# sara-nl/saraGAN

Hardware: AMD Instinct MI355X
Metric: 3D volumes/sec/node (G+D step) at 128x128x32 (higher is better)
Workload: dtype bf16

## Files before the change

### saragan_amd/csrc/common.h

```cpp
#pragma once
#include <hip/hip_runtime.h>
#include <stdint.h>
#include <mutex>
#include "../../include/saragan_hip.h"

typedef __bf16 bf16_t;
typedef float f32x4 __attribute__((ext_vector_type(4)));
typedef float f32x16 __attribute__((ext_vector_type(16)));
typedef __bf16 bf16x8 __attribute__((ext_vector_type(8)));
typedef __bf16 bf16x4 __attribute__((ext_vector_type(4)));
typedef short s16x4 __attribute__((ext_vector_type(4)));
typedef uint32_t u32x4 __attribute__((ext_vector_type(4)));

#define SG_STORE16_GUARD(v) asm volatile("s_nop 1" ::"v"(v))
typedef uint32_t u32x2 __attribute__((ext_vector_type(2)));

#define SG_LAUNCH_CHECK()                          \
  do {                                             \
    hipError_t e__ = hipGetLastError();            \
    if (e__ != hipSuccess) return (int)e__;        \
  } while (0)

static inline hipStream_t sg_st(sg_stream_t s) { return (hipStream_t)s; }

struct sg_config {
  int fwd_lds, fwd_tg;
  int fwd_v1, fwd_no_pw, fwd_no_dense;
  int fwd_no_v3, fwd_no_v3s, fwd_no_v4, fwd_no_v5, fwd_no_ksplit;
  int fwd3p_16;
  int fwd3s_16;
  int fwd_no_3p;
  int fwd3_gx, fwd3_no_lean;
  int fwd4_gx, fwd4_no_lean, fwd4_no_wres;
  int wgrad_v1, wgrad_no_v3, wgrad_no_lean;
  int wgrad_no_w16;
  int wgrad3l_min_cols;
  int wgrad3l_16;
  int wgrad_v1_blocks;
  int dbg_flags;
  int no_small;
  int deterministic;
  int gemm_ks_model;
  int gemm_k333_maxvox;
  int no_gemm;
};
const sg_config& sg_cfg();

bool sg_gemm_conv_eligible(const sg_conv_shape* s, sg_dtype dt);
size_t sg_gemm_conv_workspace(const sg_conv_shape* s, sg_dtype dt);
int sg_gemm_conv_fwd(const void* x, const void* wp, void* y, const sg_conv_shape* s, const float* bias, int act, float slope,
                     const uint32_t* mask_bits, float mask_slope, uint32_t* sign_out, void* workspace, size_t workspace_bytes,
                     hipStream_t st, bool* used);

bool sg_small_eligible(const sg_conv_shape* s);
bool sg_small_wgrad_eligible(const sg_conv_shape* s);
size_t sg_small_tail_bytes(const sg_conv_shape* s);
size_t sg_small_wgrad_workspace(const sg_conv_shape* s);
int sg_small_pack(const float* w, float coef, int flip, void* tail, const sg_conv_shape* s, sg_dtype dt, hipStream_t st);
int sg_small_fwd(const void* x, const void* tail, void* y, const sg_conv_shape* s, const float* bias, int act, float slope,
                 int pixel_norm, float eps, float* pn_scale, const uint32_t* mask_bits, float mask_slope, uint32_t* sign_out,
                 sg_dtype dt, hipStream_t st);
int sg_small_wgrad(const void* x, const void* dy, float* dw, float* dbias, float coef, void* workspace, size_t workspace_bytes,
                   const sg_conv_shape* s, sg_dtype dt, hipStream_t st);

#define SG_ALLOW_160K_LDS(kern)                                                                                  \
  do {                                                                                                           \
    static std::once_flag once__;                                                                                \
    static hipError_t err__ = hipSuccess;                                                                        \
    std::call_once(once__, [&] {                                                                                 \
      err__ = hipFuncSetAttribute((const void*)(kern), hipFuncAttributeMaxDynamicSharedMemorySize, 160 * 1024);  \
    });                                                                                                          \
    if (err__ != hipSuccess) return (int)err__;                                                                  \
  } while (0)
static inline size_t sg_esize(sg_dtype dt) { return dt == SG_BF16 ? 2 : 4; }
static inline bool sg_aligned16(const void* p) { return (((uintptr_t)p) & 15) == 0; }

__device__ __forceinline__ void philox4x32_10(uint32_t c0, uint32_t c1, uint32_t c2, uint32_t c3, uint32_t k0,
                                              uint32_t k1, uint32_t out[4]) {
#pragma unroll
  for (int rnd = 0; rnd < 10; ++rnd) {
    const uint32_t hi0 = __umulhi(0xD2511F53u, c0), lo0 = 0xD2511F53u * c0;
    const uint32_t hi1 = __umulhi(0xCD9E8D57u, c2), lo1 = 0xCD9E8D57u * c2;
    const uint32_t n0 = hi1 ^ c1 ^ k0, n1 = lo1, n2 = hi0 ^ c3 ^ k1, n3 = lo0;
    c0 = n0; c1 = n1; c2 = n2; c3 = n3;
    k0 += 0x9E3779B9u; k1 += 0xBB67AE85u;
  }
  out[0] = c0; out[1] = c1; out[2] = c2; out[3] = c3;
}

struct sg_fastdiv {
  uint32_t d, m;
};
static inline __host__ __device__ sg_fastdiv sg_make_fastdiv(uint32_t d) {
  sg_fastdiv f;
  f.d = d;
  f.m = d <= 1 ? 0u : (uint32_t)((0x100000000ull + d - 1) / d);
  return f;
}
__device__ __forceinline__ uint32_t sg_div(uint32_t x, sg_fastdiv f) {
  return f.d <= 1 ? x : __umulhi(x, f.m);
}

template <typename T>
struct sg_traits;
template <>
struct sg_traits<float> {
  static constexpr int CH = 8;
  __device__ static __forceinline__ float to_f(float v) { return v; }
  __device__ static __forceinline__ float from_f(float v) { return v; }
};
template <>
struct sg_traits<bf16_t> {
  static constexpr int CH = 16;
  __device__ static __forceinline__ float to_f(bf16_t v) { return (float)v; }
  __device__ static __forceinline__ bf16_t from_f(float v) { return (bf16_t)v; }
};

template <typename T>
__device__ __forceinline__ f32x16 sg_mfma_chunk(u32x4 a, u32x4 b, f32x16 c);
template <>
// ... 201 lines not shown
```

### saragan_amd/csrc/prof.hip

```cpp
#include "prof.h"
#include <mutex>
#include <vector>
#include <string.h>
#include <stdlib.h>
#include <atomic>

namespace {
struct Rec { int kind; sg_conv_shape shape; int dtype; hipEvent_t e0, e1; bool ok; const char* name; };
std::mutex g_mu;
bool g_on = false;
bool g_filter = false;
int g_fkind = 0;
sg_conv_shape g_fshape;
std::vector<Rec> g_recs;
const char* kVersion = "saragan_hip 0.4 (gfx950)";
}

bool sg_prof_on() { return g_on; }
thread_local const char* sg_tls_kernel = "";

namespace {
std::atomic<const sg_config*> g_cfg{nullptr};
int env_int(const char* name, int dflt) {
  const char* v = getenv(name);
  return v && *v ? atoi(v) : dflt;
}
const sg_config* read_config() {
  sg_config* c = new sg_config;
  c->fwd_lds = env_int("SG_FWD_LDS", 80 * 1024);
  c->fwd_tg = env_int("SG_FWD_TG", 0);
  c->fwd_v1 = env_int("SG_FWD_V1", 0);
  c->fwd_no_pw = env_int("SG_FWD_NO_PW", 0);
  c->fwd_no_dense = env_int("SG_FWD_NO_DENSE", 0);
  c->fwd_no_v3 = env_int("SG_FWD_NO_V3", 0);
  c->fwd_no_v3s = env_int("SG_FWD_NO_V3S", 0);
  c->wgrad_no_lean = env_int("SG_WGRAD_NO_LEAN", 0);
  c->wgrad_no_w16 = env_int("SG_WGRAD_NO_W16", 0);
  c->wgrad3l_16 = env_int("SG_WGRAD3L_16", 0);
  c->wgrad3l_min_cols = env_int("SG_WGRAD3L_MIN_COLS", 0);
  c->wgrad_v1_blocks = env_int("SG_WGRAD_V1_BLOCKS", 0);
  c->fwd_no_v4 = env_int("SG_FWD_NO_V4", 0);
  c->fwd_no_v5 = env_int("SG_FWD_NO_V5", 0);
  c->fwd_no_ksplit = env_int("SG_FWD_NO_KSPLIT", 0);
  c->fwd_no_3p = env_int("SG_FWD_NO_3P", 0);
  c->fwd3p_16 = env_int("SG_FWD3P_16", 1);
  c->fwd3s_16 = env_int("SG_FWD3S_16", 1);
  c->fwd3_gx = env_int("SG_FWD3_GX", 0);
  c->fwd3_no_lean = env_int("SG_FWD3_NO_LEAN", 0);
  c->fwd4_gx = env_int("SG_FWD4_GX", 0);
  c->fwd4_no_lean = env_int("SG_FWD4_NO_LEAN", 0);
  c->fwd4_no_wres = env_int("SG_FWD4_NO_WRES", 0);
  c->wgrad_v1 = env_int("SG_WGRAD_V1", 0);
  c->wgrad_no_v3 = env_int("SG_WGRAD_NO_V3", 0);
  c->dbg_flags = env_int("SG_DBG_FLAGS", 0);
  c->no_small = env_int("SG_NO_SMALL", 0);
  c->deterministic = env_int("SG_DETERMINISTIC", 0);
  c->no_gemm = env_int("SG_NO_GEMM", 0);
  c->gemm_ks_model = env_int("SG_GEMM_KS_MODEL", 0);
  c->gemm_k333_maxvox = env_int("SG_GEMM_K333_MAXVOX", 8192);
  return c;
}
}

const sg_config& sg_cfg() {
  const sg_config* c = g_cfg.load(std::memory_order_acquire);
  if (c == nullptr) {
    std::lock_guard<std::mutex> lk(g_mu);
    c = g_cfg.load(std::memory_order_acquire);
    if (c == nullptr) {
      c = read_config();
      g_cfg.store(c, std::memory_order_release);
    }
  }
  return *c;
}

extern "C" int sg_config_reload(void) {
  std::lock_guard<std::mutex> lk(g_mu);
  g_cfg.store(read_config(), std::memory_order_release);
  return SG_OK;
}

void sg_prof_begin(int kind, const sg_conv_shape* s, sg_dtype dt, hipStream_t st, int* slot) {
  std::lock_guard<std::mutex> lk(g_mu);
  if (g_filter && (kind != g_fkind || memcmp(s, &g_fshape, sizeof(sg_conv_shape)) != 0)) { *slot = -1; return; }
  Rec r; r.kind = kind; r.shape = *s; r.dtype = (int)dt; r.ok = false; r.name = "";
  if (hipEventCreate(&r.e0) != hipSuccess) { *slot = -1; return; }
  if (hipEventCreate(&r.e1) != hipSuccess) { (void)hipEventDestroy(r.e0); *slot = -1; return; }
  (void)hipEventRecord(r.e0, st);
  g_recs.push_back(r);
  *slot = (int)g_recs.size() - 1;
}

void sg_prof_end(int slot, hipStream_t st) {
  std::lock_guard<std::mutex> lk(g_mu);
  bool ok = slot >= 0;
  int idx = ok ? slot : -1 - slot;
  if (idx < 0 || idx >= (int)g_recs.size()) return;
  (void)hipEventRecord(g_recs[idx].e1, st);
  g_recs[idx].ok = ok;
}

void sg_prof_name(int slot, const char* name) {
  std::lock_guard<std::mutex> lk(g_mu);
  if (slot >= 0 && slot < (int)g_recs.size()) g_recs[slot].name = name;
}

extern "C" const char* sg_version(void) { return kVersion; }

extern "C" const char* sg_error_string(int code) {
  switch (code) {
    case SG_OK: return "ok";
    case SG_EINVAL: return "invalid argument (shape, null pointer or unsupported combination)";
    case SG_EWORKSPACE: return "workspace too small";
    case SG_EALIGN: return "pointer not 16-byte aligned";
    case SG_EUNSUPPORTED: return "no kernel covers this request";
    default: break;
  }
  if (code > 0) return hipGetErrorString((hipError_t)code);
  return "unknown error";
}
// ... 53 lines not shown
```

### saragan_amd/csrc/wgrad.hip

```cpp
#include "common.h"
#include "prof.h"
#include <stdlib.h>
#include <type_traits>

struct WgradArgs {
  const void* x;
  const void* dy;
  float* dwt;
  sg_tile_geom g;
  sg_tile_geom gy;
  int cin, cout, taps, kh, kw, tap0, taps_blk;
  int ciT, coT;
  int rs;
  int xbytes, ybytes;
  int ntiles;
  sg_fastdiv fnp;
  int vec_x, vec_y;
  int plane_rows;
  float* dbias;
  int64_t slab, bslab;
  int nslab;
  int dbg_flags;
  unsigned long long* dbg;
  const uint32_t* dy_mask;
// ... 967 lines not shown
  template <int I>
  static __device__ __forceinline__ void prologue(const Ctx& c, frag_t (&a0)[RING], frag_t (&a1)[RING], frag_t (&b0)[2],
                                                  frag_t (&b1)[2]) {
    if constexpr (I < PF && I < NI) {
      load<I>(c, a0, a1, b0, b1);
      prologue<I + 1>(c, a0, a1, b0, b1);
    }
  }
  static __device__ __forceinline__ void run(const Ctx& c, f32x16 (&acc)[MAXT]) {
    frag_t a0[RING], a1[RING], b0[2], b1[2];
    SG_KLOOP_BEGIN();
    prologue<0>(c, a0, a1, b0, b1);
    step<0>(c, acc, a0, a1, b0, b1);
    SG_KLOOP_END();
  }
};

template <int PF, int TW = 32>
struct sg_wgrad_tile_lean16 {
  static constexpr int MAXT = 7, TH = 128 / TW, HW = TW + 2, RPS = 32 / TW;
  static constexpr int NKS = 8, IPS = 2 + 2 * MAXT, NI = NKS * IPS, RING = PF + 1;
  static_assert(PF * 2 + 2 <= 15, "lgkmcnt is a 4-bit counter");
  typedef s16x4 frag_t;
  struct Ctx {
    int xb[2][MAXT];
    int yb;
  };
  struct HF { frag_t p[2]; };
  template <int I>
  static __device__ __forceinline__ void load(const Ctx& c, HF (&a)[RING], HF (&b)[2][2]) {
    constexpr int ks = I / IPS, r = I % IPS, td = ks / (NKS / 2), th = (ks % (NKS / 2)) * RPS;
    if constexpr (r < 2) {
      asm volatile("ds_read_b64_tr_b16 %0, %1 offset:%2" : "=v"(b[ks & 1][r].p[0]) : "v"(c.yb), "n"(ks * 2048 + r * 32));
      asm volatile("ds_read_b64_tr_b16 %0, %1 offset:%2" : "=v"(b[ks & 1][r].p[1]) : "v"(c.yb), "n"(ks * 2048 + r * 32 + 256));
    } else {
      constexpr int t = r - 2, j = t / 2, h = t % 2, SL = (ks * 2 * MAXT + t) % RING;
      constexpr int off = th * HW * 64 + h * 32;
      asm volatile("ds_read_b64_tr_b16 %0, %1 offset:%2" : "=v"(a[SL].p[0]) : "v"(c.xb[td][j]), "n"(off));
      asm volatile("ds_read_b64_tr_b16 %0, %1 offset:%2" : "=v"(a[SL].p[1]) : "v"(c.xb[td][j]), "n"(off + 256));
    }
  }
  static __device__ __forceinline__ u32x4 cat(const HF& f) {
    u32x4 o;
    o[0] = __builtin_bit_cast(u32x2, f.p[0])[0]; o[1] = __builtin_bit_cast(u32x2, f.p[0])[1];
    o[2] = __builtin_bit_cast(u32x2, f.p[1])[0]; o[3] = __builtin_bit_cast(u32x2, f.p[1])[1];
    return o;
  }
  template <int I>
  static __device__ __forceinline__ void step(const Ctx& c, f32x4 (&acc)[MAXT][4], HF (&a)[RING], HF (&b)[2][2]) {
    if constexpr (I < NI) {
      if constexpr (I + PF < NI) load<I + PF>(c, a, b);
      constexpr int ks = I / IPS, r = I % IPS;
      if constexpr (r >= 2) {
        constexpr int younger = (NI - 1 - I < PF ? NI - 1 - I : PF) * 2;
        asm volatile("s_waitcnt lgkmcnt(%0)" ::"n"(younger));
        __builtin_amdgcn_sched_barrier(0);
        constexpr int t = r - 2, j = t / 2, h = t % 2, SL = (ks * 2 * MAXT + t) % RING;
        const u32x4 af = cat(a[SL]);
#pragma unroll
        for (int hb = 0; hb < 2; ++hb)
          acc[j][h * 2 + hb] = __builtin_amdgcn_mfma_f32_16x16x32_bf16(__builtin_bit_cast(bf16x8, af), __builtin_bit_cast(bf16x8, cat(b[ks & 1][hb])),
                                                                       acc[j][h * 2 + hb], 0, 0, 0);
        __builtin_amdgcn_sched_barrier(0);
      }
      step<I + 1>(c, acc, a, b);
    }
  }
  template <int I>
  static __device__ __forceinline__ void prologue(const Ctx& c, HF (&a)[RING], HF (&b)[2][2]) {
    if constexpr (I < PF && I < NI) {
      load<I>(c, a, b);
      prologue<I + 1>(c, a, b);
    }
  }
  static __device__ __forceinline__ void run(const Ctx& c, f32x4 (&acc)[MAXT][4]) {
    HF a[RING], b[2][2];
    SG_KLOOP_BEGIN();
    prologue<0>(c, a, b);
    step<0>(c, acc, a, b);
    SG_KLOOP_END();
  }
};

template <bool UPS, bool DYM = false, int TW = 32, bool M16 = false>
__global__ __launch_bounds__(512) void conv_wgrad3l_kernel(WgradArgs a) {
  static_assert(!(UPS && DYM), "one gathered operand at a time");
  static_assert(TW == 32 || TW == 16, "tile width");
  extern __shared__ __attribute__((aligned(16))) char smem[];
  constexpr int TAPS = 27, MAXT = 7;
  constexpr int TH = 128 / TW, HH = TH + 2, HW = TW + 2, PB = 208 * 64, XB = 4 * PB, YB = 256 * 64, BUF = XB + YB;
  static_assert(HH * HW <= 208, "halo plane slot");
  constexpr int XPIECES = (HH * HW + 15) / 16;
  constexpr int ONES_OFF = 2 * BUF, ONES_BYTES = 12288;
  static_assert((TH - 1) * HW * 64 + 2304 + 1024 + 12 * 64 + 64 <= ONES_BYTES, "ones image covers every fragment offset");
  for (int i = threadIdx.x * 16; i < ONES_BYTES; i += 512 * 16)
    *reinterpret_cast<u32x4*>(smem + ONES_OFF + i) = u32x4{0x3F803F80u, 0x3F803F80u, 0x3F803F80u, 0x3F803F80u};
  constexpr uint32_t DEAD = 0x80000000u;
  const sg_tile_geom& g = a.g;
  const int tid = threadIdx.x, lane = tid & 63;
  const int wave8 = __builtin_amdgcn_readfirstlane(tid >> 6);
  const int grp = wave8 >> 2, wave = wave8 & 3;
  const int xmine = grp * BUF, ymine = xmine + XB;
  const int ci_t = blockIdx.y / a.coT, co_t = blockIdx.y % a.coT;
  const int D = g.D, H = g.H, W = g.W, nTd = g.nTd, cin = a.cin, cout = a.cout;

  const int ncol = g.nTn * g.nTh * g.nTw;
  const int xg = blockIdx.x & 7, bslot = blockIdx.x >> 3;
  const int per_x = gridDim.x >> 3;
  const int cpx = (ncol + 7) >> 3;
  const int c_begin = xg * cpx, c_end = min(ncol, c_begin + cpx);
  const int cfirst = c_begin + bslot;
  const int ncols_blk = cfirst < c_end ? (c_end - cfirst + per_x - 1) / per_x : 0;
  const int ncols_mine = (ncols_blk + 1 - grp) >> 1;
  const int items_mine = ncols_mine * nTd;
  const int items_max = ((ncols_blk + 1) >> 1) * nTd;

  const int i16 = lane & 15, q16 = lane >> 4;
  const int qd = i16 >> 2, pp = i16 & 3;
  const int colb = M16 ? 4 * pp * 2 : (16 * (q16 & 1) + 4 * pp) * 2;
  const int kb = M16 ? 8 * (q16 & 1) + qd : 8 * (q16 >> 1) + qd;
  const int xl0 = xmine + kb * 64 + colb + (M16 ? (q16 >> 1) * (TW == 32 ? 1024 : HW * 64) : 0);
  const int yl0 = ymine + kb * 64 + colb + (M16 ? (q16 >> 1) * 1024 : 0);

  constexpr int MAXP = 4, MAXY = 4;
  uint32_t relx[MAXP], rely[MAXY], relm[DYM ? MAXY : 1];
  int crdx[MAXP], crdy[MAXY];
#pragma unroll
  for (int k = 0; k < MAXP; ++k) {
    const int it = (wave + 4 * k) * 64 + lane;
    const int row = it >> 2, c = ci_t * 32 + (it & 3) * 8;
    const int hh_ = row / HW, hw = row - hh_ * HW;
    const bool live = row < HH * HW && c < cin && (wave + 4 * k) < XPIECES;
    const int rel = UPS ? ((((hh_ - 1) >> 1) * (W >> 1) + ((hw - 1) >> 1)) * cin + c) * 2 : ((hh_ * W + hw) * cin + c) * 2;
    relx[k] = live ? (uint32_t)rel : 0xC0000000u;
    crdx[k] = live ? (hw | (hh_ << 8)) : 0x7F7F;
  }
#pragma unroll
  for (int k = 0; k < MAXY; ++k) {
    const int it = (wave + 4 * k) * 64 + lane;
    const int row = it >> 2, c = co_t * 32 + (it & 3) * 8;
    const int tw = row & (TW - 1), th = (row / TW) & (TH - 1), td = row >> 7;
    if constexpr (DYM) {
      rely[k] = c < cout ? (uint32_t)(((((th >> 1) * (W >> 1)) + (tw >> 1)) * cout + c) * 2) : 0xC0000000u;
      relm[k] = c < cout ? (uint32_t)((((td * H + th) * W + tw) * a.coT + co_t) * 4 + (it & 3)) : 0xC0000000u;
    } else {
      rely[k] = c < cout ? (uint32_t)((((td * H + th) * W + tw) * cout + c) * 2) : 0xC0000000u;
    }
    crdy[k] = th;
  }
  const int64_t svox = (int64_t)D * H * W;
  const int64_t xsb = (UPS ? svox >> 3 : svox) * cin * 2, ysb = (DYM ? svox >> 3 : svox) * cout * 2, msb = svox * a.coT * 4;
  const uint32_t xplane = (uint32_t)((UPS ? (H >> 1) * (W >> 1) : H * W) * cin * 2),
                 yplane = (uint32_t)((DYM ? (H >> 1) * (W >> 1) : H * W) * cout * 2), mplane = (uint32_t)(H * W * a.coT * 4);

  int cj = 0, di = 0;
  __amdgpu_buffer_rsrc_t rx, ry, rm;
  uint32_t vkx[MAXP], vky[MAXY], vkm[DYM ? MAXY : 1];
  auto enter_column = [&]() {
    const int col = cfirst + (2 * cj + grp) * per_x;
    const int c1 = (int)sg_div((uint32_t)col, g.fnTw);
    const int w0 = (col - c1 * g.nTw) * TW;
    const int c2 = (int)sg_div((uint32_t)c1, g.fnTh);
    const int h0 = (c1 - c2 * g.nTh) * TH;
    const int n0 = c2;
    rx = __builtin_amdgcn_make_buffer_rsrc(const_cast<char*>(reinterpret_cast<const char*>(a.x)) + n0 * xsb, 0, (int)xsb, 0x00020000);
    ry = __builtin_amdgcn_make_buffer_rsrc(const_cast<char*>(reinterpret_cast<const char*>(a.dy)) + n0 * ysb, 0, (int)ysb, 0x00020000);
    if constexpr (DYM)
      rm = __builtin_amdgcn_make_buffer_rsrc(const_cast<char*>(reinterpret_cast<const char*>(a.dy_mask)) + n0 * msb, 0, (int)msb, 0x00020000);
    const int tile_off = UPS ? ((h0 >> 1) * (W >> 1) + (w0 >> 1)) * cin * 2
                             : ((h0 - 1) * W + (w0 - 1)) * cin * 2;
    const int lo_w = max(0, 1 - w0), hi_w = min(HW, W + 1 - w0) - 1;
    const int lo_h = max(0, 1 - h0), hi_h = min(HH, H + 1 - h0) - 1;
    const uint32_t lo = (uint32_t)(lo_w | (lo_h << 8));
    const uint32_t hi = (uint32_t)(hi_w | (hi_h << 8)) | 0x8080u;
#pragma unroll
    for (int k = 0; k < MAXP; ++k) {
      const uint32_t c_ = (uint32_t)crdx[k];
      const uint32_t t1 = (c_ | 0x8080u) - lo, t2 = hi - c_;
      vkx[k] = (t1 & t2 & 0x8080u) == 0x8080u ? relx[k] + (uint32_t)tile_off : DEAD;
    }
    const int col_off = DYM ? ((h0 >> 1) * (W >> 1) + (w0 >> 1)) * cout * 2 : (h0 * W + w0) * cout * 2;
    const int rows_left = H - h0;
#pragma unroll
    for (int k = 0; k < MAXY; ++k) {
      const bool in = crdy[k] < rows_left && rely[k] < DEAD;
      vky[k] = in ? rely[k] + (uint32_t)col_off : DEAD;
      if constexpr (DYM) vkm[k] = in ? relm[k] + (uint32_t)((h0 * W + w0) * a.coT * 4) : DEAD;
    }
  };
  const float gain_y = a.dy_gain, slope_y = a.dy_mask_slope;
  auto stage = [&]() __attribute__((always_inline)) {
    const int d0 = 2 * di;
    u32x4 sy[DYM ? MAXY : 1];
    uint32_t my[DYM ? MAXY : 1];
    if constexpr (DYM) {
      const uint32_t ysoff = (uint32_t)(d0 >> 1) * yplane, msoff = (uint32_t)d0 * mplane;
#pragma unroll
      for (int k = 0; k < MAXY; ++k) {
        const bool ok = d0 + (k >> 1) < D;
        sy[k] = __builtin_amdgcn_raw_buffer_load_b128(ry, ok ? vky[k] : DEAD, ysoff, 0);
        my[k] = __builtin_amdgcn_raw_buffer_load_b8(rm, ok ? vkm[k] : DEAD, msoff, 0);
      }
    }
#pragma unroll
    for (int hd = 0; hd < 4; ++hd) {
      if (hd < 2 && di != 0) continue;
      const int gp = d0 - 1 + hd;
      const bool plane_ok = gp >= 0 && gp < D;
      const uint32_t soff = plane_ok ? (uint32_t)(UPS ? gp >> 1 : gp) * xplane : 0u;
      char* dst = smem + xmine + ((gp + 8) & 3) * PB;
#pragma unroll
      for (int k = 0; k < MAXP; ++k)
        if (wave + 4 * k < XPIECES)
          __builtin_amdgcn_raw_ptr_buffer_load_lds(rx, (lds_ptr_t)(dst + (wave + 4 * k) * 1024), 16, plane_ok ? vkx[k] : DEAD, soff, 0, 0);
    }
    if constexpr (DYM) {
#pragma unroll
      for (int k = 0; k < MAXY; ++k)
        *reinterpret_cast<u32x4*>(smem + ymine + (wave + 4 * k) * 1024 + lane * 16) = sg_mask_piece_bf16(sy[k], my[k], gain_y, slope_y);
    } else {
      const uint32_t ysoff = (uint32_t)d0 * yplane;
#pragma unroll
      for (int k = 0; k < MAXY; ++k) {
        const bool ok = d0 + (k >> 1) < D;
        __builtin_amdgcn_raw_ptr_buffer_load_lds(ry, (lds_ptr_t)(smem + ymine + (wave + 4 * k) * 1024), 16, ok ? vky[k] : DEAD, ysoff, 0, 0);
      }
    }
  };
  auto advance = [&]() {
    if (++di == nTd) {
      di = 0;
      ++cj;
      if (cj < ncols_mine) enter_column();
    }
  };

  int tap_hw[MAXT], tap_kd[MAXT];
#pragma unroll
  for (int j = 0; j < MAXT; ++j) {
    const int tap = wave + 4 * j;
    const int kw_i = tap % 3, kh_i = (tap / 3) % 3, kd_i = tap / 9;
    tap_hw[j] = tap < TAPS ? (kh_i * HW + kw_i) * 64 : 0;
    tap_kd[j] = tap < TAPS ? kd_i : 0;
  }
  const int ones_last = (a.dbias != nullptr && ci_t == 0 && wave == 3) ? 1 : 0;
  typename std::conditional<M16, f32x4[MAXT][4], f32x16[MAXT]>::type acc;
#pragma unroll
  for (int j = 0; j < MAXT; ++j)
#pragma unroll
    for (int i = 0; i < 16; ++i) {
      if constexpr (M16) acc[j][i >> 2][i & 3] = 0.f;
      else acc[j][i] = 0.f;
    }

  int dbgi = 0;
  auto stamp = [&]() {
    if (a.dbg != nullptr && blockIdx.x == 8 && blockIdx.y == 0 && lane == 0 && wave == 0 && dbgi < 120)
      a.dbg[grp * 128 + dbgi] = __builtin_amdgcn_s_memtime();
    ++dbgi;
  };
  typedef typename std::conditional<M16, sg_wgrad_tile_lean16<5, TW>, sg_wgrad_tile_lean<5, TW>>::type KT;
  auto mfma_phase = [&](int q) {
    const int dq = q % nTd;
    const int pbase = 2 * dq - 1 + 8;
    typename KT::Ctx c;
    c.yb = yl0;
#pragma unroll
    for (int td = 0; td < 2; ++td)
#pragma unroll
      for (int j = 0; j < MAXT; ++j) c.xb[td][j] = xl0 + ((pbase + td + tap_kd[j]) & 3) * PB + tap_hw[j];
    if (ones_last) c.xb[0][MAXT - 1] = c.xb[1][MAXT - 1] = ONES_OFF + (xl0 - xmine);
    KT::run(c, acc);
  };
  const bool stage_first_only = (a.dbg_flags & 1) != 0;
  auto off_phase = [&](int qn) {
    if (qn < items_mine && !(stage_first_only && qn >= 1)) stage();
    stamp();
    if (qn < items_mine) advance();
    asm volatile("s_waitcnt vmcnt(0)" ::: "memory");
  };

  if (items_mine > 0) enter_column();
  if (grp == 0) {
    off_phase(0);
    __syncthreads();
    for (int q = 0; q < items_max; ++q) {
      stamp();
      if (q < items_mine) mfma_phase(q);
      stamp();
      __syncthreads();
      stamp();
      off_phase(q + 1);
      stamp();
      __syncthreads();
    }
  } else {
    __syncthreads();
    for (int q = 0; q < items_max; ++q) {
      stamp();
      off_phase(q);
      stamp();
      __syncthreads();
      stamp();
      if (q < items_mine) mfma_phase(q);
      stamp();
      __syncthreads();
    }
  }
  {
    char* cbuf = smem + ((wave * MAXT) << 12) + lane * 16;
    if (grp == 1) {
#pragma unroll
      for (int j = 0; j < MAXT; ++j)
#pragma unroll
        for (int i4 = 0; i4 < 4; ++i4) {
          if constexpr (M16) *reinterpret_cast<f32x4*>(cbuf + ((j * 4 + i4) << 10)) = acc[j][i4];
          else *reinterpret_cast<f32x4*>(cbuf + ((j * 4 + i4) << 10)) = f32x4{acc[j][4 * i4], acc[j][4 * i4 + 1], acc[j][4 * i4 + 2], acc[j][4 * i4 + 3]};
        }
    }
    __syncthreads();
    if (grp == 1) return;
#pragma unroll
    for (int j = 0; j < MAXT; ++j)
#pragma unroll
      for (int i4 = 0; i4 < 4; ++i4) {
        const f32x4 o = *reinterpret_cast<const f32x4*>(cbuf + ((j * 4 + i4) << 10));
#pragma unroll
        for (int e = 0; e < 4; ++e) {
          if constexpr (M16) acc[j][i4][e] += o[e];
          else acc[j][4 * i4 + e] += o[e];
        }
      }
  }
  if constexpr (M16) {
    const int c16 = lane & 15, q4 = lane >> 4;
    if (ones_last && (items_mine > 0 || a.slab != 0) && q4 == 0) {
#pragma unroll
      for (int hb = 0; hb < 2; ++hb)
        if (co_t * 32 + 16 * hb + c16 < cout)
          sg_wg_out(a.dbias + (int64_t)blockIdx.x * a.bslab + co_t * 32 + 16 * hb + c16, acc[MAXT - 1][hb][0], a.slab != 0);
    }
#pragma unroll
    for (int j = 0; j < MAXT; ++j) {
      const int tap = wave + 4 * j;
      if (tap < TAPS && (items_mine > 0 || a.slab != 0)) {
        float* dst = a.dwt + (int64_t)blockIdx.x * a.slab + ((((int64_t)tap * a.ciT + ci_t) * a.coT + co_t) << 10);
#pragma unroll
        for (int t = 0; t < 4; ++t)
#pragma unroll
          for (int e = 0; e < 4; ++e)
            sg_wg_out(dst + (16 * (t >> 1) + 4 * q4 + e) * 32 + 16 * (t & 1) + c16, acc[j][t][e], a.slab != 0);
      }
    }
  } else {
    const int r = lane & 31, hh = lane >> 5;
    if (ones_last && (items_mine > 0 || a.slab != 0) && hh == 0 && co_t * 32 + r < cout)
      sg_wg_out(a.dbias + (int64_t)blockIdx.x * a.bslab + co_t * 32 + r, acc[MAXT - 1][0], a.slab != 0);
#pragma unroll
    for (int j = 0; j < MAXT; ++j) {
      const int tap = wave + 4 * j;
      if (tap < TAPS && (items_mine > 0 || a.slab != 0)) {
        float* dst = a.dwt + (int64_t)blockIdx.x * a.slab + ((((int64_t)tap * a.ciT + ci_t) * a.coT + co_t) << 10);
#pragma unroll
        for (int i = 0; i < 16; ++i) {
          const int row = (i & 3) + 8 * (i >> 2) + 4 * hh;
          sg_wg_out(dst + row * 32 + r, acc[j][i], a.slab != 0);
        }
      }
    }
  }
}

template <int KD, int KH, int KW>
static int launch_wgrad3(WgradArgs& a, const sg_conv_shape* s, hipStream_t st, bool* used) {
  *used = false;
  const bool w16 = KD == 3 && KH == 3 && KW == 3 && s->w == 16 && (s->h % 8) == 0 && (s->d % 2) == 0 && !a.dy_mask &&
                   !sg_cfg().wgrad_no_lean && !sg_cfg().wgrad_no_w16;
  a.g = sg_make_geom(s, 256, true, 2, w16 ? 8 : 4);
  const sg_tile_geom& g = a.g;
  if (g.TW != (w16 ? 16 : 32) || g.TN != 1 || g.TD * g.TH * g.TW != 256) return SG_OK;
  if (g.HD != 2 && g.HD != 4) return SG_OK;
  if (g.TD != 2 || g.TH != (w16 ? 8 : 4)) return SG_OK;
  if (g.HH > 127 || g.HW > 127) return SG_OK;
  if ((s->cin % 8) || (s->cout % 8)) return SG_OK;
  if ((int64_t)g.TN * s->d * s->h * s->w * (int64_t)(s->cin > s->cout ? s->cin : s->cout) >= (1ll << 31)) return SG_OK;
  const int ncol = g.nTn * g.nTh * g.nTw;
  const int pairs = a.ciT * a.coT;
  int gx = (256 / pairs) / 8 * 8;
  if (gx < 8) gx = 8;
  while (gx > 8 && ncol < 2 * gx && (gx - 8) * pairs >= (w16 ? 128 : 64)) gx -= 8;
  const int min_cols = sg_cfg().wgrad3l_min_cols > 0 ? sg_cfg().wgrad3l_min_cols : 2;
  if (ncol < (2 * gx < min_cols ? 2 * gx : min_cols) || g.nTd < 2) return SG_OK;
  a.gy = a.g;
  a.ntiles = ncol * g.nTd;
  a.rs = 64;
  a.plane_rows = (g.HH * g.HW + 15) & ~15;
  if (a.plane_rows / 16 > 16) return SG_OK;
  a.xbytes = g.HD * a.plane_rows * 64;
  a.ybytes = 256 * 64;
  size_t lds = 2ull * (a.xbytes + a.ybytes);
  if (lds > 160 * 1024) return SG_OK;
  a.tap0 = 0; a.taps_blk = a.taps;
  a.nslab = 2 * gx;
  const bool lean = KD == 3 && KH == 3 && KW == 3 && g.HH == 6 && g.HW == 34 && g.HD == 4 && a.plane_rows == 208 &&
                    s->w % 32 == 0 && !sg_cfg().wgrad_no_lean && (!g.ups || ((s->d | s->h | s->w) & 1) == 0);
  const bool lean16 = w16 && g.HH == 10 && g.HW == 18 && g.HD == 4 && (!g.ups || ((s->d | s->h | s->w) & 1) == 0);
  if (w16 && !lean16) return SG_OK;
  if (lean16 || lean) a.nslab = gx;
  if (lean) lds += 12288;
  const bool m16 = sg_cfg().wgrad3l_16 != 0;
#define SG_LAUNCH_WGRAD3L(UPS_, DYM_, TW_, NAME_)                                                                     \
  do {                                                                                                               \
    if (m16) {                                                                                                       \
      auto kern = conv_wgrad3l_kernel<UPS_, DYM_, TW_, true>;                                                        \
      SG_ALLOW_160K_LDS(kern);                                                                                       \
      SG_KNAME(NAME_);                                                                                               \
      hipLaunchKernelGGL(kern, dim3((unsigned)gx, (unsigned)pairs), dim3(512), lds, st, a);                          \
    } else {                                                                                                         \
      auto kern = conv_wgrad3l_kernel<UPS_, DYM_, TW_, false>;                                                       \
      SG_ALLOW_160K_LDS(kern);                                                                                       \
      SG_KNAME(NAME_);                                                                                               \
      hipLaunchKernelGGL(kern, dim3((unsigned)gx, (unsigned)pairs), dim3(512), lds, st, a);                          \
    }                                                                                                                \
  } while (0)
  if (lean16) {
    lds = 2ull * (4 * 208 * 64 + 256 * 64) + 12288;
    if (g.ups) SG_LAUNCH_WGRAD3L(true, false, 16, "conv_wgrad3l<ups,w16>");
    else SG_LAUNCH_WGRAD3L(false, false, 16, "conv_wgrad3l<w16>");
  } else if (a.dy_mask) {
    if (!lean || g.ups || ((s->d | s->h | s->w) & 1)) return SG_OK;
    SG_LAUNCH_WGRAD3L(false, true, 32, "conv_wgrad3l<dy gather>");
  } else if (lean && g.ups) {
    SG_LAUNCH_WGRAD3L(true, false, 32, "conv_wgrad3l<ups>");
  } else if (lean) {
    SG_LAUNCH_WGRAD3L(false, false, 32, "conv_wgrad3l");
#undef SG_LAUNCH_WGRAD3L
  } else {
    auto kern = conv_wgrad3_kernel<KD, KH, KW>;
    SG_ALLOW_160K_LDS(kern);
    SG_KNAME("conv_wgrad3<%d,%d,%d>", KD, KH, KW);
    hipLaunchKernelGGL(kern, dim3((unsigned)gx, (unsigned)pairs), dim3(512), lds, st, a);
  }
  SG_LAUNCH_CHECK();
  *used = true;
  return SG_OK;
}

struct WgradPlanesArgs {
  const void* x;
  const void* dy;
  float* dwt;
  float* dbias;
  int cin, cout, ciT, coT;
  int ntiles;
  int64_t slab, bslab;
};

template <int HW_>
__device__ __forceinline__ void conv_wgrad_planes_body(const WgradPlanesArgs& a) {
  extern __shared__ __attribute__((aligned(16))) char smem[];
  constexpr int H = HW_, W = HW_, P = 128 / (H * W), RP = (H + 2) * (W + 2);
  constexpr int XROWS = P * RP, NPX = (XROWS * 4 + 255) / 256, NPY = 2, PPT = NPX + NPY;
  constexpr int XB = NPX * 4096, YB = 128 * 64, BUF = XB + YB;
  constexpr uint32_t DEAD = 0x80000000u;
  const int tid = threadIdx.x, lane = tid & 63;
  const int wave = __builtin_amdgcn_readfirstlane(tid >> 6);
  const int ci_t = blockIdx.y / a.coT, co_t = blockIdx.y % a.coT;
  const int cin = a.cin, cout = a.cout;
  uint32_t vx[NPX], vy[NPY];
#pragma unroll
  for (int k = 0; k < NPX; ++k) {
    const int it = tid + 256 * k;
    const int row = it >> 2, sub = it & 3;
    const int p = row / RP, rr = row - p * RP;
    const int hh = rr / (W + 2), hw = rr - hh * (W + 2);
    const bool in = row < XROWS && hh >= 1 && hh <= H && hw >= 1 && hw <= W;
    vx[k] = in ? (uint32_t)((((p * H + hh - 1) * W + hw - 1) * cin + ci_t * 32 + sub * 8) * 2) : DEAD;
  }
#pragma unroll
  for (int k = 0; k < NPY; ++k) {
    const int it = tid + 256 * k;
    vy[k] = (uint32_t)(((it >> 2) * cout + co_t * 32 + (it & 3) * 8) * 2);
  }
  const __amdgpu_buffer_rsrc_t rx = __builtin_amdgcn_make_buffer_rsrc(const_cast<void*>(a.x), 0, (int)((int64_t)a.ntiles * 128 * cin * 2), 0x00020000);
  const __amdgpu_buffer_rsrc_t ry = __builtin_amdgcn_make_buffer_rsrc(const_cast<void*>(a.dy), 0, (int)((int64_t)a.ntiles * 128 * cout * 2), 0x00020000);
  auto stage = [&](int t, int b) __attribute__((always_inline)) {
    const bool ok = t < a.ntiles;
    const uint32_t sx = ok ? (uint32_t)t * (uint32_t)(128 * cin * 2) : 0u, sy = ok ? (uint32_t)t * (uint32_t)(128 * cout * 2) : 0u;
    char* xb = smem + b * BUF;
#pragma unroll
    for (int k = 0; k < NPX; ++k)
      __builtin_amdgcn_raw_ptr_buffer_load_lds(rx, (lds_ptr_t)(xb + (tid + 256 * k) * 16 - lane * 16), 16, ok ? vx[k] : DEAD, sx, 0, 0);
#pragma unroll
    for (int k = 0; k < NPY; ++k)
      __builtin_amdgcn_raw_ptr_buffer_load_lds(ry, (lds_ptr_t)(xb + XB + (tid + 256 * k) * 16 - lane * 16), 16, ok ? vy[k] : DEAD, sy, 0, 0);
  };
  const int i16 = lane & 15, q16 = lane >> 4;
  const int colb = (16 * (q16 & 1) + 4 * (i16 & 3)) * 2;
  const int kb = 8 * (q16 >> 1) + (i16 >> 2);
  int xr[2], yr[2];
#pragma unroll
  for (int j = 0; j < 2; ++j) {
    const int m = kb + 4 * j;
    xr[j] = ((m / W + (wave < 3 ? wave : 0)) * (W + 2) + m % W) * 64 + colb;
    yr[j] = XB + m * 64 + colb;
  }
  const bool ones = wave == 3 && a.dbias != nullptr && ci_t == 0;
  f32x16 acc[3];
#pragma unroll
  for (int j = 0; j < 3; ++j)
#pragma unroll
    for (int i = 0; i < 16; ++i) acc[j][i] = 0.f;
  const u32x4 one8 = {0x3F803F80u, 0x3F803F80u, 0x3F803F80u, 0x3F803F80u};

  typedef s16x4 __attribute__((address_space(3))) * lds_s16x4_p;
  const int t0 = blockIdx.x, G = gridDim.x;
  stage(t0, 0);
  stage(t0 + G, 1);
  int b = 0;
// ... 272 lines not shown
```

Baseline: 613.6.

## Reassign wgrad taps per wave so x rows are reused across kh taps

Adds a row-reuse inner loop for the lean 3x3x3 weight-gradient kernel. Each wave now owns taps that share kd and kw but differ in kh, so a single LDS read of an x row feeds up to three MFMAs against different dy rows. The change is enabled by default through a new env knob. It is meant to cut LDS transposed-read traffic per MFMA, at the cost of a more complex tap-to-wave mapping, a dy register ring and extra template instantiations.

```diff
diff --git a/saragan_amd/csrc/common.h b/saragan_amd/csrc/common.h
--- a/saragan_amd/csrc/common.h
+++ b/saragan_amd/csrc/common.h
@@ -36,6 +36,7 @@
   int wgrad_no_w16;
   int wgrad3l_min_cols;
   int wgrad3l_16;
+  int wgrad3l_reuse;
   int wgrad_v1_blocks;
   int dbg_flags;
   int no_small;
diff --git a/saragan_amd/csrc/prof.hip b/saragan_amd/csrc/prof.hip
--- a/saragan_amd/csrc/prof.hip
+++ b/saragan_amd/csrc/prof.hip
@@ -37,6 +37,7 @@
   c->wgrad_no_lean = env_int("SG_WGRAD_NO_LEAN", 0);
   c->wgrad_no_w16 = env_int("SG_WGRAD_NO_W16", 0);
   c->wgrad3l_16 = env_int("SG_WGRAD3L_16", 0);
+  c->wgrad3l_reuse = env_int("SG_WGRAD3L_REUSE", 1);
   c->wgrad3l_min_cols = env_int("SG_WGRAD3L_MIN_COLS", 0);
   c->wgrad_v1_blocks = env_int("SG_WGRAD_V1_BLOCKS", 0);
   c->fwd_no_v4 = env_int("SG_FWD_NO_V4", 0);
diff --git a/saragan_amd/csrc/wgrad.hip b/saragan_amd/csrc/wgrad.hip
--- a/saragan_amd/csrc/wgrad.hip
+++ b/saragan_amd/csrc/wgrad.hip
@@ -1073,7 +1073,198 @@
   }
 };
 
-template <bool UPS, bool DYM = false, int TW = 32, bool M16 = false>
+template <int PF, int TW = 32>
+struct sg_wgrad_tile_reuse {
+  static constexpr int MAXT = 7, TH = 128 / TW, HW = TW + 2, KPL = TW / 16, NBLK = 2 * KPL, ROWS = TH + 2;
+  static constexpr int IPB = 4 * TH + 4, XPB = 3 * TH + 4, NI = NBLK * IPB, RING = PF + 1, YRING = 4;
+  static constexpr int XREADS = NBLK * XPB, YREADS = NBLK * TH, MFMAS = NBLK * TH * MAXT;
+  static_assert(XREADS <= (TW == 32 ? 64 : 56) && YREADS == 16 && MFMAS == 112, "read budget of the row-reuse loop");
+  static_assert((ROWS - 1) * HW * 64 + (KPL - 1) * 1024 + 256 < 65536, "kh lives in the 16-bit instruction offset");
+  static_assert(PF * 2 <= 15, "lgkmcnt is a 4-bit counter");
+  static_assert(PF <= 5, "the dy ring of four rows");
+  typedef s16x4 frag_t;
+  struct Ctx {
+    int xb[2][3];
+    int yb;
+  };
+  struct It { int blk, r, kind, xi; };
+  static constexpr It item(int I) {
+    const int blk = I / IPB, q = I % IPB;
+    if (q < 4 * TH) return It{blk, q / 4, q % 4, blk * XPB + (q / 4) * 3 + (q % 4) - 1};
+    return It{blk, TH + (q - 4 * TH) / 2, 1 + (q - 4 * TH) % 2, blk * XPB + 3 * TH + (q - 4 * TH)};
+  }
+  template <int I>
+  static __device__ __forceinline__ void load(const Ctx& c, frag_t (&a0)[RING], frag_t (&a1)[RING], frag_t (&b0)[YRING],
+                                              frag_t (&b1)[YRING]) {
+    constexpr It it = item(I);
+    constexpr int td = it.blk / KPL, half = it.blk % KPL;
+    if constexpr (it.kind == 0) {
+      constexpr int ks = (td * TH + it.r) * KPL + half;
+      asm volatile("ds_read_b64_tr_b16 %0, %1 offset:%2" : "=v"(b0[it.r % YRING]) : "v"(c.yb), "n"(ks * 1024));
+      asm volatile("ds_read_b64_tr_b16 %0, %1 offset:%2" : "=v"(b1[it.r % YRING]) : "v"(c.yb), "n"(ks * 1024 + 256));
+    } else {
+      constexpr int SL = it.xi % RING, off = it.r * HW * 64 + half * 1024;
+      asm volatile("ds_read_b64_tr_b16 %0, %1 offset:%2" : "=v"(a0[SL]) : "v"(c.xb[td][it.kind - 1]), "n"(off));
+      asm volatile("ds_read_b64_tr_b16 %0, %1 offset:%2" : "=v"(a1[SL]) : "v"(c.xb[td][it.kind - 1]), "n"(off + 256));
+    }
+  }
+  static __device__ __forceinline__ u32x4 cat(const frag_t& lo, const frag_t& hi) {
+    u32x4 o;
+    o[0] = __builtin_bit_cast(u32x2, lo)[0]; o[1] = __builtin_bit_cast(u32x2, lo)[1];
+    o[2] = __builtin_bit_cast(u32x2, hi)[0]; o[3] = __builtin_bit_cast(u32x2, hi)[1];
+    return o;
+  }
+  template <int J, int T>
+  static __device__ __forceinline__ void mm(f32x16 (&acc)[MAXT], const u32x4& af, frag_t (&b0)[YRING], frag_t (&b1)[YRING]) {
+    acc[J] = __builtin_amdgcn_mfma_f32_32x32x16_bf16(__builtin_bit_cast(bf16x8, af),
+                                                    __builtin_bit_cast(bf16x8, cat(b0[T % YRING], b1[T % YRING])), acc[J], 0, 0, 0);
+  }
+  template <int I>
+  static __device__ __forceinline__ void step(const Ctx& c, f32x16 (&acc)[MAXT], frag_t (&a0)[RING], frag_t (&a1)[RING],
+                                              frag_t (&b0)[YRING], frag_t (&b1)[YRING]) {
+    if constexpr (I < NI) {
+      if constexpr (I + PF < NI) load<I + PF>(c, a0, a1, b0, b1);
+      constexpr It it = item(I);
+      if constexpr (it.kind != 0) {
+        constexpr int younger = (NI - 1 - I < PF ? NI - 1 - I : PF) * 2;
+        asm volatile("s_waitcnt lgkmcnt(%0)" ::"n"(younger));
+        __builtin_amdgcn_sched_barrier(0);
+        constexpr int SL = it.xi % RING;
+        const u32x4 af = cat(a0[SL], a1[SL]);
+        if constexpr (it.kind == 3) {
+          mm<6, it.r>(acc, af, b0, b1);
+        } else {
+          constexpr int j0 = (it.kind - 1) * 3;
+          if constexpr (it.r < TH) mm<j0, it.r>(acc, af, b0, b1);
+          if constexpr (it.r >= 1 && it.r - 1 < TH) mm<j0 + 1, it.r - 1>(acc, af, b0, b1);
+          if constexpr (it.r >= 2) mm<j0 + 2, it.r - 2>(acc, af, b0, b1);
+        }
+        __builtin_amdgcn_sched_barrier(0);
+      }
+      step<I + 1>(c, acc, a0, a1, b0, b1);
+    }
+  }
+  template <int I>
+  static __device__ __forceinline__ void prologue(const Ctx& c, frag_t (&a0)[RING], frag_t (&a1)[RING], frag_t (&b0)[YRING],
+                                                  frag_t (&b1)[YRING]) {
+    if constexpr (I < PF && I < NI) {
+      load<I>(c, a0, a1, b0, b1);
+      prologue<I + 1>(c, a0, a1, b0, b1);
+    }
+  }
+  static __device__ __forceinline__ void run(const Ctx& c, f32x16 (&acc)[MAXT]) {
+    frag_t a0[RING], a1[RING], b0[YRING], b1[YRING];
+    SG_KLOOP_BEGIN();
+    prologue<0>(c, a0, a1, b0, b1);
+    step<0>(c, acc, a0, a1, b0, b1);
+    SG_KLOOP_END();
+  }
+};
+
+template <int PF>
+struct sg_wgrad_tile_reuse16 {
+  static constexpr int MAXT = 7, TH = 4, HW = 34, NBLK = 4, ROWS = TH + 2;
+  static constexpr int IPB = 5 * TH + 4, XPB = 3 * TH + 4, NI = NBLK * IPB, RING = PF + 1, YRING = 4;
+  static constexpr int XREADS = NBLK * XPB, YREADS = NBLK * 2 * TH, MFMAS = NBLK * TH * MAXT * 2;
+  static_assert(XREADS <= 64 && YREADS == 32 && MFMAS == 224, "read budget of the row-reuse loop");
+  static_assert((ROWS - 1) * HW * 64 + 32 + 256 < 65536, "kh lives in the 16-bit instruction offset");
+  static_assert(PF * 2 <= 15, "lgkmcnt is a 4-bit counter");
+  static_assert(PF <= 6, "the dy ring of four rows");
+  typedef s16x4 frag_t;
+  struct Ctx {
+    int xb[2][3];
+    int yb;
+  };
+  struct HF { frag_t p[2]; };
+  struct It { int blk, r, kind, xi; };
+  static constexpr It item(int I) {
+    const int blk = I / IPB, q = I % IPB;
+    if (q < 5 * TH) return It{blk, q / 5, q % 5, blk * XPB + (q / 5) * 3 + (q % 5) - 2};
+    return It{blk, TH + (q - 5 * TH) / 2, 2 + (q - 5 * TH) % 2, blk * XPB + 3 * TH + (q - 5 * TH)};
+  }
+  template <int I>
+  static __device__ __forceinline__ void load(const Ctx& c, HF (&a)[RING], HF (&b)[YRING][2]) {
+    constexpr It it = item(I);
+    constexpr int td = it.blk / 2, h = it.blk % 2;
+    if constexpr (it.kind < 2) {
+      constexpr int off = (td * TH + it.r) * 2048 + it.kind * 32;
+      asm volatile("ds_read_b64_tr_b16 %0, %1 offset:%2" : "=v"(b[it.r % YRING][it.kind].p[0]) : "v"(c.yb), "n"(off));
+      asm volatile("ds_read_b64_tr_b16 %0, %1 offset:%2" : "=v"(b[it.r % YRING][it.kind].p[1]) : "v"(c.yb), "n"(off + 256));
+    } else {
+      constexpr int SL = it.xi % RING, off = it.r * HW * 64 + h * 32;
+      asm volatile("ds_read_b64_tr_b16 %0, %1 offset:%2" : "=v"(a[SL].p[0]) : "v"(c.xb[td][it.kind - 2]), "n"(off));
+      asm volatile("ds_read_b64_tr_b16 %0, %1 offset:%2" : "=v"(a[SL].p[1]) : "v"(c.xb[td][it.kind - 2]), "n"(off + 256));
+    }
+  }
+  static __device__ __forceinline__ u32x4 cat(const HF& f) {
+    u32x4 o;
+    o[0] = __builtin_bit_cast(u32x2, f.p[0])[0]; o[1] = __builtin_bit_cast(u32x2, f.p[0])[1];
+    o[2] = __builtin_bit_cast(u32x2, f.p[1])[0]; o[3] = __builtin_bit_cast(u32x2, f.p[1])[1];
+    return o;
+  }
+  template <int J, int H, int T>
+  static __device__ __forceinline__ void mm(f32x4 (&acc)[MAXT][4], const u32x4& af, HF (&b)[YRING][2]) {
+#pragma unroll
+    for (int hb = 0; hb < 2; ++hb)
+      acc[J][H * 2 + hb] = __builtin_amdgcn_mfma_f32_16x16x32_bf16(__builtin_bit_cast(bf16x8, af), __builtin_bit_cast(bf16x8, cat(b[T % YRING][hb])),
+                                                                   acc[J][H * 2 + hb], 0, 0, 0);
+  }
+  template <int I>
+  static __device__ __forceinline__ void step(const Ctx& c, f32x4 (&acc)[MAXT][4], HF (&a)[RING], HF (&b)[YRING][2]) {
+    if constexpr (I < NI) {
+      if constexpr (I + PF < NI) load<I + PF>(c, a, b);
+      constexpr It it = item(I);
+      if constexpr (it.kind >= 2) {
+        constexpr int younger = (NI - 1 - I < PF ? NI - 1 - I : PF) * 2;
+        asm volatile("s_waitcnt lgkmcnt(%0)" ::"n"(younger));
+        __builtin_amdgcn_sched_barrier(0);
+        constexpr int SL = it.xi % RING, h = it.blk % 2;
+        const u32x4 af = cat(a[SL]);
+        if constexpr (it.kind == 4) {
+          mm<6, h, it.r>(acc, af, b);
+        } else {
+          constexpr int j0 = (it.kind - 2) * 3;
+          if constexpr (it.r < TH) mm<j0, h, it.r>(acc, af, b);
+          if constexpr (it.r >= 1 && it.r - 1 < TH) mm<j0 + 1, h, it.r - 1>(acc, af, b);
+          if constexpr (it.r >= 2) mm<j0 + 2, h, it.r - 2>(acc, af, b);
+        }
+        __builtin_amdgcn_sched_barrier(0);
+      }
+      step<I + 1>(c, acc, a, b);
+    }
+  }
+  template <int I>
+  static __device__ __forceinline__ void prologue(const Ctx& c, HF (&a)[RING], HF (&b)[YRING][2]) {
+    if constexpr (I < PF && I < NI) {
+      load<I>(c, a, b);
+      prologue<I + 1>(c, a, b);
+    }
+  }
+  static __device__ __forceinline__ void run(const Ctx& c, f32x4 (&acc)[MAXT][4]) {
+    HF a[RING], b[YRING][2];
+    SG_KLOOP_BEGIN();
+    prologue<0>(c, a, b);
+    step<0>(c, acc, a, b);
+    SG_KLOOP_END();
+  }
+};
+
+__host__ __device__ constexpr int sg_wg3l_tap(bool ru, int w, int j) {
+  if (!ru) return w + 4 * j;
+  if (j < 6) return ((2 * w + j / 3) / 3) * 9 + (j % 3) * 3 + (2 * w + j / 3) % 3;
+  return w < 3 ? 18 + 3 * w + 2 : 27;
+}
+constexpr bool sg_wg3l_taps_cover(bool ru) {
+  int seen[28] = {};
+  for (int w = 0; w < 4; ++w)
+    for (int j = 0; j < 7; ++j) ++seen[sg_wg3l_tap(ru, w, j)];
+  for (int t = 0; t < 28; ++t)
+    if (seen[t] != 1) return false;
+  return sg_wg3l_tap(ru, 3, 6) == 27;
+}
+static_assert(sg_wg3l_taps_cover(false) && sg_wg3l_taps_cover(true), "every tap in exactly one slot; wave 3's slot 6 spare");
+
+template <bool UPS, bool DYM = false, int TW = 32, bool M16 = false, bool RU = false>
 __global__ __launch_bounds__(512) void conv_wgrad3l_kernel(WgradArgs a) {
   static_assert(!(UPS && DYM), "one gathered operand at a time");
   static_assert(TW == 32 || TW == 16, "tile width");
@@ -1229,11 +1420,13 @@
   int tap_hw[MAXT], tap_kd[MAXT];
 #pragma unroll
   for (int j = 0; j < MAXT; ++j) {
-    const int tap = wave + 4 * j;
+    const int tap = sg_wg3l_tap(RU, wave, j);
     const int kw_i = tap % 3, kh_i = (tap / 3) % 3, kd_i = tap / 9;
     tap_hw[j] = tap < TAPS ? (kh_i * HW + kw_i) * 64 : 0;
     tap_kd[j] = tap < TAPS ? kd_i : 0;
   }
+  const int colA = 2 * wave, colB = 2 * wave + 1;
+  const int col_kd[2] = {colA / 3, colB / 3}, col_kw[2] = {(colA % 3) * 64, (colB % 3) * 64};
   const int ones_last = (a.dbias != nullptr && ci_t == 0 && wave == 3) ? 1 : 0;
   typename std::conditional<M16, f32x4[MAXT][4], f32x16[MAXT]>::type acc;
 #pragma unroll
@@ -1250,17 +1443,29 @@
       a.dbg[grp * 128 + dbgi] = __builtin_amdgcn_s_memtime();
     ++dbgi;
   };
-  typedef typename std::conditional<M16, sg_wgrad_tile_lean16<5, TW>, sg_wgrad_tile_lean<5, TW>>::type KT;
+  constexpr bool ROWS1 = RU && (!M16 || TW == 32);
+  typedef typename std::conditional<M16, typename std::conditional<ROWS1, sg_wgrad_tile_reuse16<5>, sg_wgrad_tile_lean16<5, TW>>::type,
+                                    typename std::conditional<RU, sg_wgrad_tile_reuse<5, TW>, sg_wgrad_tile_lean<5, TW>>::type>::type KT;
   auto mfma_phase = [&](int q) {
     const int dq = q % nTd;
     const int pbase = 2 * dq - 1 + 8;
     typename KT::Ctx c;
     c.yb = yl0;
-#pragma unroll
-    for (int td = 0; td < 2; ++td)
-#pragma unroll
-      for (int j = 0; j < MAXT; ++j) c.xb[td][j] = xl0 + ((pbase + td + tap_kd[j]) & 3) * PB + tap_hw[j];
-    if (ones_last) c.xb[0][MAXT - 1] = c.xb[1][MAXT - 1] = ONES_OFF + (xl0 - xmine);
+    if constexpr (ROWS1) {
+#pragma unroll
+      for (int td = 0; td < 2; ++td) {
+#pragma unroll
+        for (int s = 0; s < 2; ++s) c.xb[td][s] = xl0 + ((pbase + td + col_kd[s]) & 3) * PB + col_kw[s];
+        c.xb[td][2] = xl0 + ((pbase + td + tap_kd[MAXT - 1]) & 3) * PB + tap_hw[MAXT - 1];
+      }
+      if (ones_last) c.xb[0][2] = c.xb[1][2] = ONES_OFF + (xl0 - xmine);
+    } else {
+#pragma unroll
+      for (int td = 0; td < 2; ++td)
+#pragma unroll
+        for (int j = 0; j < MAXT; ++j) c.xb[td][j] = xl0 + ((pbase + td + tap_kd[j]) & 3) * PB + tap_hw[j];
+      if (ones_last) c.xb[0][MAXT - 1] = c.xb[1][MAXT - 1] = ONES_OFF + (xl0 - xmine);
+    }
     KT::run(c, acc);
   };
   const bool stage_first_only = (a.dbg_flags & 1) != 0;
@@ -1333,7 +1538,7 @@
     }
 #pragma unroll
     for (int j = 0; j < MAXT; ++j) {
-      const int tap = wave + 4 * j;
+      const int tap = sg_wg3l_tap(RU, wave, j);
       if (tap < TAPS && (items_mine > 0 || a.slab != 0)) {
         float* dst = a.dwt + (int64_t)blockIdx.x * a.slab + ((((int64_t)tap * a.ciT + ci_t) * a.coT + co_t) << 10);
 #pragma unroll
@@ -1349,7 +1554,7 @@
       sg_wg_out(a.dbias + (int64_t)blockIdx.x * a.bslab + co_t * 32 + r, acc[MAXT - 1][0], a.slab != 0);
 #pragma unroll
     for (int j = 0; j < MAXT; ++j) {
-      const int tap = wave + 4 * j;
+      const int tap = sg_wg3l_tap(RU, wave, j);
       if (tap < TAPS && (items_mine > 0 || a.slab != 0)) {
         float* dst = a.dwt + (int64_t)blockIdx.x * a.slab + ((((int64_t)tap * a.ciT + ci_t) * a.coT + co_t) << 10);
 #pragma unroll
@@ -1400,19 +1605,20 @@
   if (lean16 || lean) a.nslab = gx;
   if (lean) lds += 12288;
   const bool m16 = sg_cfg().wgrad3l_16 != 0;
+  const bool ru = sg_cfg().wgrad3l_reuse != 0;
+#define SG_LAUNCH_WGRAD3L_1(UPS_, DYM_, TW_, M16_, RU_, NAME_)                                                        \
+  do {                                                                                                               \
+    auto kern = conv_wgrad3l_kernel<UPS_, DYM_, TW_, M16_, RU_>;                                                     \
+    SG_ALLOW_160K_LDS(kern);                                                                                         \
+    SG_KNAME(NAME_);                                                                                                 \
+    hipLaunchKernelGGL(kern, dim3((unsigned)gx, (unsigned)pairs), dim3(512), lds, st, a);                            \
+  } while (0)
 #define SG_LAUNCH_WGRAD3L(UPS_, DYM_, TW_, NAME_)                                                                     \
   do {                                                                                                               \
-    if (m16) {                                                                                                       \
-      auto kern = conv_wgrad3l_kernel<UPS_, DYM_, TW_, true>;                                                        \
-      SG_ALLOW_160K_LDS(kern);                                                                                       \
-      SG_KNAME(NAME_);                                                                                               \
-      hipLaunchKernelGGL(kern, dim3((unsigned)gx, (unsigned)pairs), dim3(512), lds, st, a);                          \
-    } else {                                                                                                         \
-      auto kern = conv_wgrad3l_kernel<UPS_, DYM_, TW_, false>;                                                       \
-      SG_ALLOW_160K_LDS(kern);                                                                                       \
-      SG_KNAME(NAME_);                                                                                               \
-      hipLaunchKernelGGL(kern, dim3((unsigned)gx, (unsigned)pairs), dim3(512), lds, st, a);                          \
-    }                                                                                                                \
+    if (m16 && ru) SG_LAUNCH_WGRAD3L_1(UPS_, DYM_, TW_, true, true, NAME_);                                          \
+    else if (m16) SG_LAUNCH_WGRAD3L_1(UPS_, DYM_, TW_, true, false, NAME_);                                          \
+    else if (ru) SG_LAUNCH_WGRAD3L_1(UPS_, DYM_, TW_, false, true, NAME_);                                           \
+    else SG_LAUNCH_WGRAD3L_1(UPS_, DYM_, TW_, false, false, NAME_);                                                  \
   } while (0)
   if (lean16) {
     lds = 2ull * (4 * 208 * 64 + 256 * 64) + 12288;
@@ -1426,6 +1632,7 @@
   } else if (lean) {
     SG_LAUNCH_WGRAD3L(false, false, 32, "conv_wgrad3l");
 #undef SG_LAUNCH_WGRAD3L
+#undef SG_LAUNCH_WGRAD3L_1
   } else {
     auto kern = conv_wgrad3_kernel<KD, KH, KW>;
     SG_ALLOW_160K_LDS(kern);
```

After: 620.0 (median of 6 runs). 1.01x the previous value.
